# researchaccelerator-hub/distributed-crawler

Hardware: NVIDIA H100
Metric: messages/sec parsed+link-extracted+JSONL (higher is better)
Workload: dtype u8

## Files before the change

distributed_crawler_b200/csrc/kernels.cuh:

```cuda
#pragma once
#include "scalars.cuh"
#include "tg_walk.cuh"
#include "tg_lane.cuh"
#include "yt_walk.cuh"
#include "gm_walk.cuh"
#include "yt_lane.cuh"

namespace tgi {

constexpr int WARPS_PER_CTA = 8;
constexpr int CTA_THREADS = WARPS_PER_CTA * 32;
#ifndef LB_PARSE
#define LB_PARSE 6
#endif
#ifndef LB_SIZE
#define LB_SIZE 6
#endif
#ifndef LB_ESC
#define LB_ESC 6
#endif
#ifndef LB_MAPS
#define LB_MAPS 6
#endif
#ifndef LB_YT
// ... 79 lines not shown
  TgRecView v;
  const tgi_tg_rec* rec = &b.recs[r];
  v.rec = rec;
  v.text = b.strs + rec->str_off;
  v.text_len = rec->text_len;
  v.alt = v.text + v.text_len;
  v.alt_len = rec->alt_len;
  v.media = v.alt + v.alt_len;
  v.media_len = rec->media_len;
  v.handle = v.media + v.media_len;
  v.handle_len = rec->handle_len;
  v.ct = rec->content_type;
  v.flags = rec->flags;
  v.e0 = b.ent_off[r];
  v.e1 = b.ent_off[r + 1];
  return v;
}

template <bool ENTITIES>
DEVI void parse_one_record(const TgBatchDev& b, const CfgDev& cfg, const ParseOut& o, uint64_t r, TgRecView v) {
  const int l = lane_id();
  uint32_t status = TGI_ST_EMITTED, nlinks = 0, lstart = 0;
  if ((cfg.flags & TGI_CFG_HAS_MIN_POST_DATE) && (int64_t)v.rec->date < cfg.min_post_date) {
    status = TGI_ST_SKIPPED;
  } else if (v.flags & TGI_RF_PANIC) {
    status = TGI_ST_FAILED;
  } else {
    if (!ENTITIES) v.e1 = v.e0;
    uint32_t ub = warp_link_upper_bound(v, b.ents);
    if (ub >= (1u << 20)) {
      if (l == 0) atomicOr(o.err, ERR_TOO_MANY_LINKS);
      ub = 0;
    }
    if (ub) {
      if (l == 0) lstart = atomicAdd(o.cursor, ub);
      lstart = __shfl_sync(FULL, lstart, 0);
      if (lstart + ub > o.arena_cap || lstart + ub < lstart) {
        if (l == 0) atomicOr(o.err, ERR_ARENA_OVERFLOW);
      } else {
        const tgi_tg_chan* ch = &b.chans[v.rec->chan_idx];
        LinkSink ls;
        ls.out = o.arena + lstart;
        ls.cap = ub;
        ls.count = 0;
        ls.name_bytes = 0;
        ls.self = b.chan_strs + ch->str_off + ch->title_len;
        ls.self_len = ch->name_len;
        bool ok = warp_extract_links(v, b.ents, b.aux, o.ent_range, ls);
        nlinks = ls.count;
        if (!ok) {
          status = TGI_ST_FAILED;
          nlinks = 0;
        }
      }
    }
  }
  if (l == 0) {
    o.status[r] = (uint8_t)status;
    o.linelen[r] = 0;
    o.link_start[r] = lstart;
    o.link_count[r] = nlinks;
  }
}

DEVI void tg_parse_body(const TgBatchDev& b, const CfgDev& cfg, uint32_t run_flags, const ParseOut& o) {
  int wid = threadIdx.x >> 5;
  uint64_t nwarps = (uint64_t)gridDim.x * WARPS_PER_CTA;
  for (uint64_t r = (uint64_t)blockIdx.x * WARPS_PER_CTA + wid; r < b.n; r += nwarps) {
    const uint64_t rn = r + nwarps;
    unsigned long long nx_off = 0;
    uint32_t nx_len = 0;
    if (rn < b.n) {
      asm volatile("ld.global.nc.u64 %0, [%1];" : "=l"(nx_off) : "l"(&b.recs[rn].str_off));
      asm volatile("ld.global.nc.u32 %0, [%1];" : "=r"(nx_len) : "l"(&b.recs[rn].text_len));
    }
    if (b.ent_off[r + 1] == b.ent_off[r])
      parse_one_record<false>(b, cfg, o, r, load_rec_view(b, r));
    if (rn < b.n) {
      const uint32_t off = (uint32_t)lane_id() * 128u;
      if (off < nx_len + 127u && off < 2048u) asm volatile("prefetch.global.L1 [%0];" ::"l"(b.strs + nx_off + off));
    }
  }
}
__global__ void __launch_bounds__(CTA_THREADS, LB_PARSE) tg_parse_kernel(TgBatchDev b, CfgDev cfg, uint32_t run_flags, ParseOut o) { tg_parse_body(b, cfg, run_flags, o); }
DEVI void tg_ent_map_body(const TgBatchDev& b, const ParseOut& o) {
  const int wid = threadIdx.x >> 5, l = lane_id();
  const uint64_t ngroups = (b.n + 31) / 32, nwarps = (uint64_t)gridDim.x * WARPS_PER_CTA;
  for (uint64_t g = (uint64_t)blockIdx.x * WARPS_PER_CTA + wid; g < ngroups; g += nwarps) {
    const uint64_t rl = g * 32 + l;
    uint32_t todo = __ballot_sync(FULL, rl < b.n && b.ent_off[rl + 1] != b.ent_off[rl]);
    while (todo) {
      const uint64_t r = g * 32 + (uint32_t)(__ffs(todo) - 1);
      todo &= todo - 1;
      warp_map_entities(load_rec_view(b, r), b.ents, o.ent_range);
    }
  }
}
__global__ void __launch_bounds__(CTA_THREADS, LB_PARSE) tg_ent_map_kernel(TgBatchDev b, ParseOut o) { tg_ent_map_body(b, o); }
DEVI void tg_parse_ent_body(const TgBatchDev& b, const CfgDev& cfg, uint32_t run_flags, const ParseOut& o) {
  const int wid = threadIdx.x >> 5, l = lane_id();
  const uint64_t ngroups = (b.n + 31) / 32, nwarps = (uint64_t)gridDim.x * WARPS_PER_CTA;
  for (uint64_t g = (uint64_t)blockIdx.x * WARPS_PER_CTA + wid; g < ngroups; g += nwarps) {
    const uint64_t rl = g * 32 + l;
    uint32_t todo = __ballot_sync(FULL, rl < b.n && b.ent_off[rl + 1] != b.ent_off[rl]);
    while (todo) {
      const uint64_t r = g * 32 + (uint32_t)(__ffs(todo) - 1);
      todo &= todo - 1;
      parse_one_record<true>(b, cfg, o, r, load_rec_view(b, r));
    }
  }
}
__global__ void __launch_bounds__(CTA_THREADS, LB_PARSE) tg_parse_ent_kernel(TgBatchDev b, CfgDev cfg, uint32_t run_flags, ParseOut o) {
  tg_parse_ent_body(b, cfg, run_flags, o);
}

DEVI void tg_size_lane_body(const TgBatchDev& b, const CfgDev& cfg, const ParseOut& o) {
  const int wid = threadIdx.x >> 5, l = lane_id();
  const uint64_t ngroups = (b.n + 31) / 32, nwarps = (uint64_t)gridDim.x * WARPS_PER_CTA;
  uint64_t var_sum = 0;
  for (uint64_t g = (uint64_t)blockIdx.x * WARPS_PER_CTA + wid; g < ngroups; g += nwarps) {
    uint64_t r = g * 32 + l;
    bool active = r < b.n;
    if (!active) r = b.n - 1;
    active = active && o.status[r] == TGI_ST_EMITTED;
    if (!__any_sync(FULL, active)) continue;
    TgWalkArgs a;
    a.b = &b;
    a.cfg = &cfg;
    a.r = r;
    a.v = load_rec_view(b, r);
    a.links = o.arena + o.link_start[r];
    a.n_links = active ? o.link_count[r] : 0u;
    const tgi_tg_rec* rec = a.v.rec;
    const ChanDerived cd = b.chan_derived[rec->chan_idx];
    const TgDerived d = tg_derive(a, cd);
    uint32_t xl[8] = {0, 0, 0, 0, 0, 0, 0, 0};
    uint32_t tot = 0;
    bool warp_comments = false, warp_map = false;
    const uint32_t r0 = b.react_off[r], nr = b.react_off[r + 1] - r0;
    if (active && !(cfg.flags & CFGDEV_CLOCK_INVALID)) {
      uint32_t L[8] = {ndigits_i64(rec->id / 1048576), ndigits_i64(rec->chat_id), ndigits_i64(rec->view_count),
                       ndigits_i64(rec->share_count), ndigits_i64(d.ncomments), cfg.tz == 0 ? 22u : 27u, 0, 0};
      uint32_t chan[4] = {cd.user_len, cd.name_len, cd.title_len, cd.cdata_len};
      uint32_t cf[4] = {cfg.label_len, cfg.created_tg_len, cfg.created_yt_len, cfg.capture_len};
      tot = tg_size_fixed(L, chan, cf, d.has_user, d.album);
      tot += a.v.ct == TGI_CT_OTHER ? 0u : (uint32_t)kPostTypeLen[a.v.ct];
      if (a.v.ct == TGI_CT_OTHER) xl[XL_ALT] = thread_esc_len(a.v.alt, a.v.alt_len);
      if (d.has_media) xl[XL_MEDIA] = thread_esc_len(a.v.media, a.v.media_len);
      xl[XL_HANDLE] = thread_esc_len(a.v.handle, a.v.handle_len);
      if (d.comments_nil) xl[XL_COMMENTS] = 4;
      else if (d.c1 == d.c0) xl[XL_COMMENTS] = 2;
      else warp_comments = true;
      if (nr == 0) {
        xl[XL_REACTIONS] = 2;
        xl[XL_FLAGS] = XLF_SIMPLE_MAP;
      } else if (nr <= LANE_MAP_MAX) {
        uint32_t sz = 2u, live = 0;
        bool simple = true;
        for (uint32_t j = 0; j < nr; j++) {
          const tgi_reaction rc = b.reacts[r0 + j];
          const uint8_t* kp = b.aux + rc.emoji_off;
          const uint32_t el = thread_esc_len(kp, rc.emoji_len);
          simple = simple && el == rc.emoji_len && rc.emoji_len >= 1 && rc.emoji_len <= 8;
          bool last = true;
          for (uint32_t i = j + 1; i < nr; i++) {
            const tgi_reaction ri = b.reacts[r0 + i];
            if (key_cmp(b.aux + ri.emoji_off, ri.emoji_len, kp, rc.emoji_len) == 0) last = false;
          }
          if (last) {
            sz += 3u + el + ndigits_i64(rc.count);
            live++;
          }
        }
        if (simple) {
          xl[XL_REACTIONS] = sz + (live - 1u);
          xl[XL_FLAGS] = XLF_SIMPLE_MAP;
        } else {
          warp_map = true;
        }
      } else {
        warp_map = true;
      }
      if (a.n_links) {
        uint32_t s = a.n_links - 1u;
        for (uint32_t k = 0; k < a.n_links; k++) s += a.links[k].len + 2u;
        xl[XL_OUTLINKS] = s;
      }
    }
    const bool sized = active && !(cfg.flags & CFGDEV_CLOCK_INVALID);
    uint32_t todo = __ballot_sync(FULL, sized && d.desc_len != 0);
    while (todo) {
      const int src = __ffs(todo) - 1;
      todo &= todo - 1;
      const uint8_t* p = (const uint8_t*)__shfl_sync(FULL, (unsigned long long)(uintptr_t)d.desc, src);
      const uint32_t n = __shfl_sync(FULL, d.desc_len, src);
      bool ex = false;
      const uint32_t e = warp_esc_len(p, n, &ex);
      if (l == src) {
        xl[XL_DESC] = e;
        if (ex) xl[XL_FLAGS] |= XLF_DESC_EXACT;
      }
    }
    todo = __ballot_sync(FULL, warp_comments);
    while (todo) {
      const int src = __ffs(todo) - 1;
      todo &= todo - 1;
      const uint32_t e = size_tg_comments(b, __shfl_sync(FULL, d.c0, src), __shfl_sync(FULL, d.c1, src));
      if (l == src) xl[XL_COMMENTS] = e;
    }
    todo = __ballot_sync(FULL, warp_map);
    while (todo) {
      const int src = __ffs(todo) - 1;
      todo &= todo - 1;
      const uint32_t q0 = __shfl_sync(FULL, r0, src), qn = __shfl_sync(FULL, nr, src);
      uint32_t simple = 0;
      const uint32_t e = size_reaction_map(b.reacts, q0, q0 + qn, b.aux, &simple);
      if (l == src) {
        xl[XL_REACTIONS] = e;
        xl[XL_FLAGS] = (xl[XL_FLAGS] & ~XLF_SIMPLE_MAP) | (simple ? XLF_SIMPLE_MAP : 0u);
      }
    }
    if (active) {
      uint32_t var = 0;
#pragma unroll
      for (int j = 0; j < XL_COUNT; j++) var += xl[j];
      const uint32_t llen = sized ? tot + var : 0u;
      *(uint4*)(o.xlen + r * 8) = make_uint4(xl[0], xl[1], xl[2], xl[3]);
      *(uint4*)(o.xlen + r * 8 + 4) = make_uint4(xl[4], xl[5], xl[6], xl[7]);
      if (llen == 0) o.status[r] = TGI_ST_NOLINE;
      o.linelen[r] = llen;
      if (llen) var_sum += var;
    }
  }
  for (int dd = 16; dd; dd >>= 1) var_sum += __shfl_down_sync(FULL, var_sum, dd);
  if (l == 0 && var_sum) atomicAdd(o.var_total, (unsigned long long)var_sum);
}
__global__ void __launch_bounds__(CTA_THREADS, LB_SIZE) tg_size_lane_kernel(TgBatchDev b, CfgDev cfg, ParseOut o) { tg_size_lane_body(b, cfg, o); }

struct EmitIn {
  const uint8_t* status;
  const uint64_t* line_off;
  const uint32_t* link_start;
  const uint32_t* link_count;
  const uint32_t* xlen;
  uint32_t* xpos;
  const tgi_link* arena;
  uint8_t* out;
  int* err;
  uint32_t lane_text_max;
  unsigned long long* counters;
  uint32_t* list[3];
  uint32_t* list_count;
};
enum { WL_SPARSE = 0, WL_DENSE = 1, WL_MAPS = 2 };
DEVI void wl_append(uint32_t* list, uint32_t* count, bool need, uint32_t value) {
  const uint32_t m = __ballot_sync(FULL, need);
  if (!m) return;
  uint32_t base = 0;
  if (lane_id() == 0) base = atomicAdd(count, (uint32_t)__popc(m));
  base = __shfl_sync(FULL, base, 0);
  if (need) list[base + __popc(m & ((1u << lane_id()) - 1u))] = value;
}

DEVI void tg_emit_lane_body(const TgBatchDev& b, const CfgDev& cfg, const EmitIn& in, LaneShared& sh) {
  static_assert(LANE_WARPS == WARPS_PER_CTA, "one field row block per warp");
  lane_shared_fill(sh);
  __syncthreads();
  const int wid = threadIdx.x >> 5, l = lane_id();
  const uint64_t ngroups = (b.n + 31) / 32, nwarps = (uint64_t)gridDim.x * WARPS_PER_CTA;
  LaneStream s;
  ls_init(s, smem_addr(sh.stage[wid][l]));
  uint64_t bytes_out = 0, bytes_in = 0;
  for (uint64_t g = (uint64_t)blockIdx.x * WARPS_PER_CTA + wid; g < ngroups; g += nwarps) {
    uint64_t r = g * 32 + l;
    bool active = r < b.n;
    if (!active) r = b.n - 1;
    active = active && in.status[r] == TGI_ST_EMITTED;
    if (!__any_sync(FULL, active)) continue;
    uint32_t left = 0;
    emit_tg_lane(sh, sh.rows[wid][l], s, b, cfg, r, active, in.out, in.line_off, in.xlen + r * 8, in.xpos + r * 8,
                 in.arena + in.link_start[r], active ? in.link_count[r] : 0u, in.err, bytes_out, bytes_in, left);
    bool sparse = false;
    if (active && (left & 1u)) {
      const tgi_tg_rec* rec = &b.recs[r];
      const uint32_t ct = rec->content_type;
      const bool text_desc = ct == TGI_CT_TEXT || ct == TGI_CT_VIDEO || ct == TGI_CT_PHOTO || ct == TGI_CT_ANIMATION;
      const uint32_t dlen = text_desc ? ((rec->flags & TGI_RF_HAS_TEXT) ? rec->text_len : 0u) : rec->alt_len;
      sparse = esc_desc_is_sparse(in.xlen[r * 8 + XL_DESC], dlen, in.xlen[r * 8 + XL_FLAGS]);
    }
    wl_append(in.list[WL_SPARSE], in.list_count + WL_SPARSE, active && sparse, (uint32_t)r);
    wl_append(in.list[WL_DENSE], in.list_count + WL_DENSE, active && (((left & 1u) && !sparse) || (left & 0xEu)), (uint32_t)r);
    wl_append(in.list[WL_MAPS], in.list_count + WL_MAPS, active && (left & 16u), (uint32_t)r);
  }
  for (int dd = 16; dd; dd >>= 1) {
    bytes_out += __shfl_down_sync(FULL, bytes_out, dd);
    bytes_in += __shfl_down_sync(FULL, bytes_in, dd);
  }
  if (l == 0) {
    atomicAdd(in.counters, (unsigned long long)bytes_out);
    atomicAdd(in.counters + 1, (unsigned long long)bytes_in);
  }
}
#ifndef LB_LANE
#define LB_LANE 3
#endif
__global__ void __launch_bounds__(CTA_THREADS, LB_LANE) tg_emit_lane_kernel(TgBatchDev b, CfgDev cfg, EmitIn in) {
  extern __shared__ __align__(128) uint8_t lane_smem[];
  tg_emit_lane_body(b, cfg, in, *(LaneShared*)lane_smem);
}

template <int MODE>
DEVI void tg_emit_esc_body(const TgBatchDev& b, const EmitIn& in) {
  const int wid = threadIdx.x >> 5;
  const uint32_t* list = in.list[MODE == ESC_SPARSE ? WL_SPARSE : WL_DENSE];
  const uint32_t cnt = in.list_count[MODE == ESC_SPARSE ? WL_SPARSE : WL_DENSE];
  const uint32_t nwarps = gridDim.x * WARPS_PER_CTA;
  for (uint32_t i = blockIdx.x * WARPS_PER_CTA + wid; i < cnt; i += nwarps) {
    const uint64_t rr = list[i];
    TgWalkArgs a;
    a.b = &b;
    a.cfg = nullptr;
    a.r = rr;
    a.v = load_rec_view(b, rr);
    emit_tg_escapes<MODE>(in.out + in.line_off[rr], a, in.xlen + rr * 8, in.xpos + rr * 8, in.lane_text_max);
  }
}
template <int MODE>
__global__ void __launch_bounds__(CTA_THREADS, LB_ESC) tg_emit_esc_kernel(TgBatchDev b, EmitIn in) { tg_emit_esc_body<MODE>(b, in); }

DEVI void tg_emit_maps_body(const TgBatchDev& b, const EmitIn& in) {
  __shared__ MapScratch mss[WARPS_PER_CTA];
  const int wid = threadIdx.x >> 5;
  const uint32_t cnt = in.list_count[WL_MAPS], nwarps = gridDim.x * WARPS_PER_CTA;
  for (uint32_t i = blockIdx.x * WARPS_PER_CTA + wid; i < cnt; i += nwarps) {
    const uint64_t r = in.list[WL_MAPS][i];
    uint8_t* line = in.out + in.line_off[r];
    const uint32_t* xp = in.xpos + r * 8;
    const bool comments_nil = (b.recs[r].flags & TGI_RF_COMMENTS_NIL) != 0;
    const uint32_t c0 = b.comment_off[r], c1 = b.comment_off[r + 1];
    if (!comments_nil && c1 != c0) emit_tg_comments(line + xp[XL_COMMENTS], &mss[wid], b, c0, c1);
    const uint32_t r0 = b.react_off[r], r1 = b.react_off[r + 1];
    if (r1 != r0 && !(in.xlen[r * 8 + XL_FLAGS] & XLF_SIMPLE_MAP)) emit_reaction_map(line + xp[XL_REACTIONS], &mss[wid], b.reacts, r0, r1, b.aux);
    const uint32_t nl = in.link_count[r];
    if (nl > LANE_LINKS_MAX) emit_tg_outlinks(line + xp[XL_OUTLINKS], in.arena + in.link_start[r], nl);
    __syncwarp();
  }
}
__global__ void __launch_bounds__(CTA_THREADS, LB_MAPS) tg_emit_maps_kernel(TgBatchDev b, EmitIn in) { tg_emit_maps_body(b, in); }

struct YtOut {
  uint8_t* status;
  uint32_t* linelen;
  uint32_t* url_start;
  uint32_t* url_count;
  YtUrl* urls;
  uint32_t urls_cap;
  uint32_t* url_cursor;
  uint32_t* esc_len;
  uint32_t* link_start;
  uint32_t* link_count;
  tgi_link* arena;
  uint32_t arena_cap;
  uint32_t* cursor;
  int* err;
};

DEVI void yt_parse_body(const YtBatchDev& b, const CfgDev& cfg, uint32_t run_flags, const YtOut& o) {
  int wid = threadIdx.x >> 5, l = lane_id();
  uint64_t nwarps = (uint64_t)gridDim.x * WARPS_PER_CTA;
  for (uint64_t r = (uint64_t)blockIdx.x * WARPS_PER_CTA + wid; r < b.n; r += nwarps) {
    const tgi_yt_rec v = b.recs[r];
    const uint8_t* desc = b.strs + v.str_off + v.id_len + v.title_len;
    uint32_t us = 0, uc = 0, ls = 0, lc = 0;
    uint32_t ub = yt_count_http(desc, v.desc_len);
    if (ub) {
      if (l == 0) us = atomicAdd(o.url_cursor, ub);
      us = __shfl_sync(FULL, us, 0);
      if (us + ub > o.urls_cap || us + ub < us) {
        if (l == 0) atomicOr(o.err, ERR_ARENA_OVERFLOW);
      } else {
        uc = yt_extract_urls(desc, v.desc_len, o.urls + us, ub);
      }
    }
    if (run_flags & (TGI_RUN_LINKS | TGI_RUN_FRONTIER)) {
      uint32_t lb = yt_count_ytcom(desc, v.desc_len);
      if (lb >= (1u << 20)) {
        if (l == 0) atomicOr(o.err, ERR_TOO_MANY_LINKS);
        lb = 0;
      }
      if (lb) {
        if (l == 0) ls = atomicAdd(o.cursor, lb);
        ls = __shfl_sync(FULL, ls, 0);
        if (ls + lb > o.arena_cap || ls + lb < ls) {
          if (l == 0) atomicOr(o.err, ERR_ARENA_OVERFLOW);
        } else {
          lc = yt_channel_ids(desc, v.desc_len, o.arena + ls, lb);
        }
      }
    }
    if (l == 0) {
      uint8_t tmp[40];
      bool ok = !(cfg.flags & CFGDEV_CLOCK_INVALID) && cfg.created_yt_len != 0 &&
                render_time(tmp, v.published_sec, v.published_nsec, 0) != 0;
      if (ok) {
        const tgi_yt_chan& ch = b.chans[v.chan_idx];
        if (ch.cached) ok = render_time(tmp, ch.published_sec, ch.published_nsec, 0) != 0;
      }
      o.status[r] = ok ? TGI_ST_EMITTED : TGI_ST_NOLINE;
      o.linelen[r] = 0;
      o.url_start[r] = us;
      o.url_count[r] = uc;
      o.link_start[r] = ls;
      o.link_count[r] = lc;
    }
  }
}
__global__ void __launch_bounds__(CTA_THREADS, LB_YT) yt_parse_kernel(YtBatchDev b, CfgDev cfg, uint32_t run_flags, YtOut o) { yt_parse_body(b, cfg, run_flags, o); }

DEVI void yt_size_record(const YtBatchDev& b, const CfgDev& cfg, const YtOut& o, uint64_t r, YtScratch* sc) {
  const int l = lane_id();
  {
    YtArgs a;
    a.b = &b;
    a.cfg = &cfg;
    a.r = r;
    a.urls = o.urls + o.url_start[r];
    a.n_urls = o.url_count[r];
    YtSizer z;
    z.sc = sc;
    {
      const tgi_yt_rec* rec = &b.recs[r];
      const uint8_t* title = b.strs + rec->str_off + rec->id_len;
      z.el[1] = warp_esc_len(title, rec->title_len);
      z.el[0] = warp_esc_len(title + rec->title_len, rec->desc_len);
    }
    bool ok = walk_yt_record(z, a);
    if (l == 0) {
      o.esc_len[3 * r] = z.el[0];
      o.esc_len[3 * r + 1] = z.el[1];
      o.esc_len[3 * r + 2] = z.dirty ? 0u : 1u;
      o.linelen[r] = ok ? (uint32_t)z.total : 0u;
      if (!ok) o.status[r] = TGI_ST_NOLINE;
    }
  }
}
__global__ void __launch_bounds__(CTA_THREADS, LB_YT) yt_size_kernel(YtBatchDev b, CfgDev cfg, YtOut o) {
  __shared__ YtScratch scs[WARPS_PER_CTA];
  int wid = threadIdx.x >> 5;
  uint64_t nwarps = (uint64_t)gridDim.x * WARPS_PER_CTA;
  for (uint64_t r = (uint64_t)blockIdx.x * WARPS_PER_CTA + wid; r < b.n; r += nwarps) {
    if (o.status[r] != TGI_ST_EMITTED) continue;
    yt_size_record(b, cfg, o, r, &scs[wid]);
  }
}

__global__ void __launch_bounds__(CTA_THREADS, LB_YT) yt_size_lane_kernel(YtBatchDev b, CfgDev cfg, YtOut o) {
  const int wid = threadIdx.x >> 5, l = lane_id();
  const uint64_t ngroups = (b.n + 31) / 32, nwarps = (uint64_t)gridDim.x * WARPS_PER_CTA;
  for (uint64_t g = (uint64_t)blockIdx.x * WARPS_PER_CTA + wid; g < ngroups; g += nwarps) {
    uint64_t r = g * 32 + l;
    bool active = r < b.n;
    if (!active) r = b.n - 1;
    active = active && o.status[r] == TGI_ST_EMITTED;
    const tgi_yt_rec* rec = &b.recs[r];
    const uint8_t* title = b.strs + rec->str_off + rec->id_len;
    const uint32_t tn = rec->title_len, dn = rec->desc_len;
    uint32_t el0 = 0, el1 = 0;
    bool exact = false;
    uint32_t todo = __ballot_sync(FULL, active);
    while (todo) {
      const int src = __ffs(todo) - 1;
      todo &= todo - 1;
      const uint8_t* t = (const uint8_t*)__shfl_sync(FULL, (unsigned long long)(uintptr_t)title, src);
      const uint32_t a = __shfl_sync(FULL, tn, src), d = __shfl_sync(FULL, dn, src);
      bool x1 = false, x0 = false;
      const uint32_t e1 = warp_esc_len(t, a, &x1), e0 = warp_esc_len(t + a, d, &x0);
      if (l == src) {
        el0 = e0;
        el1 = e1;
        exact = x0 || x1;
      }
    }
    if (!active) continue;
    YtArgs a;
    a.b = &b;
    a.cfg = &cfg;
    a.r = r;
    a.urls = o.urls + o.url_start[r];
    a.n_urls = o.url_count[r];
    YtLaneSizer z;
    z.el[0] = el0;
    z.el[1] = el1;
    const bool ok = walk_yt_record(z, a);
    o.esc_len[3 * r] = el0;
    o.esc_len[3 * r + 1] = el1;
    o.esc_len[3 * r + 2] = !z.dirty ? 1u : (!z.small_dirty && !exact) ? 2u : 0u;
    o.linelen[r] = ok ? (uint32_t)z.total : 0u;
    if (!ok) o.status[r] = TGI_ST_NOLINE;
  }
}

DEVI void yt_emit_record(const YtBatchDev& b, const CfgDev& cfg, const YtOut& o, const uint64_t* line_off, uint8_t* out, int* err,
                         uint64_t r, YtScratch* sc) {
  YtArgs a;
  a.b = &b;
  a.cfg = &cfg;
  a.r = r;
  a.urls = o.urls + o.url_start[r];
  a.n_urls = o.url_count[r];
  YtWriter w;
  w.sc = sc;
  w.el[0] = o.esc_len[3 * r];
  w.el[1] = o.esc_len[3 * r + 1];
  w.p = out + line_off[r];
  walk_yt_record(w, a);
  if (lane_id() == 0 && (uint64_t)(w.p - out) != line_off[r + 1]) atomicOr(err, ERR_LINE_MISMATCH);
  __syncwarp();
}
__global__ void __launch_bounds__(CTA_THREADS, LB_YT) yt_emit_kernel(YtBatchDev b, CfgDev cfg, YtOut o, const uint64_t* line_off, uint8_t* out, int* err,
                                                                 int lane_mode) {
  __shared__ YtScratch scs[WARPS_PER_CTA];
  int wid = threadIdx.x >> 5, l = lane_id();
  const uint64_t ngroups = (b.n + 31) / 32, nwarps = (uint64_t)gridDim.x * WARPS_PER_CTA;
  for (uint64_t g = (uint64_t)blockIdx.x * WARPS_PER_CTA + wid; g < ngroups; g += nwarps) {
    const uint64_t rl = g * 32 + l;
    uint32_t todo = __ballot_sync(FULL, rl < b.n && o.status[rl] == TGI_ST_EMITTED && !(lane_mode && o.esc_len[3 * rl + 2]));
    while (todo) {
      const uint64_t r = g * 32 + (uint32_t)(__ffs(todo) - 1);
      todo &= todo - 1;
      yt_emit_record(b, cfg, o, line_off, out, err, r, &scs[wid]);
    }
  }
}

__global__ void __launch_bounds__(CTA_THREADS, LB_YT) yt_emit_lane_kernel(YtBatchDev b, CfgDev cfg, YtOut o, const uint64_t* line_off, uint8_t* out, int* err) {
  const int wid = threadIdx.x >> 5, l = lane_id();
  const uint64_t ngroups = (b.n + 31) / 32, nwarps = (uint64_t)gridDim.x * WARPS_PER_CTA;
  for (uint64_t g = (uint64_t)blockIdx.x * WARPS_PER_CTA + wid; g < ngroups; g += nwarps) {
    const uint64_t r = g * 32 + l;
    const bool active = r < b.n && o.status[r] == TGI_ST_EMITTED && o.esc_len[3 * r + 2];
    YtLaneWriter w;
    if (active) {
      w.el[0] = o.esc_len[3 * r];
      w.el[1] = o.esc_len[3 * r + 1];
      YtArgs a;
      a.b = &b;
      a.cfg = &cfg;
      a.r = r;
      a.urls = o.urls + o.url_start[r];
      a.n_urls = o.url_count[r];
      w.begin((uint64_t)(uintptr_t)out + line_off[r]);
      walk_yt_record(w, a);
      w.end();
      if (w.s.pos != (uint64_t)(uintptr_t)out + line_off[r + 1]) atomicOr(err, ERR_LINE_MISMATCH);
    }
    __syncwarp();
    w.flush_pending(active);
  }
}

DEVI uint64_t join_hash(long long chat, long long msg) {
  uint64_t x = (uint64_t)chat * 0x9E3779B97F4A7C15ull ^ (uint64_t)msg;
  x ^= x >> 30; x *= 0xBF58476D1CE4E5B9ull;
  x ^= x >> 27; x *= 0x94D049BB133111EBull;
  return x ^ (x >> 31);
}
__global__ void join_build_kernel(const longlong2* a, uint64_t na, uint32_t* table, uint64_t mask) {
  const uint64_t i = (uint64_t)blockIdx.x * blockDim.x + threadIdx.x;
  if (i >= na) return;
  const longlong2 k = a[i];
  for (uint64_t s = join_hash(k.x, k.y) & mask;; s = (s + 1) & mask) {
    uint32_t cur = atomicCAS(&table[s], 0u, (uint32_t)i + 1u);
    if (cur == 0) return;
    const longlong2 o = a[cur - 1];
    if (o.x == k.x && o.y == k.y) {
      atomicMin(&table[s], (uint32_t)i + 1u);
      return;
    }
  }
}
__global__ void join_probe_kernel(const longlong2* a, const uint32_t* table, uint64_t mask, const longlong2* b, uint64_t nb, long long* out) {
  const uint64_t i = (uint64_t)blockIdx.x * blockDim.x + threadIdx.x;
  if (i >= nb) return;
  const longlong2 k = b[i];
  long long res = -1;
  for (uint64_t s = join_hash(k.x, k.y) & mask;; s = (s + 1) & mask) {
    const uint32_t cur = table[s];
    if (cur == 0) break;
    const longlong2 o = a[cur - 1];
    if (o.x == k.x && o.y == k.y) {
      res = (long long)cur - 1;
      break;
    }
  }
  out[i] = res;
}

__global__ void __launch_bounds__(CTA_THREADS, 4) gm_size_kernel(GmBatchDev b, CfgDev cfg, uint8_t* status, uint32_t* linelen) {
  __shared__ YtScratch scs[WARPS_PER_CTA];
  int wid = threadIdx.x >> 5, l = lane_id();
  uint64_t nwarps = (uint64_t)gridDim.x * WARPS_PER_CTA;
  for (uint64_t r = (uint64_t)blockIdx.x * WARPS_PER_CTA + wid; r < b.n; r += nwarps) {
    YtSizer z;
    z.sc = &scs[wid];
    bool ok = walk_gm_record(z, b, cfg, r);
    if (l == 0) {
      status[r] = ok ? TGI_ST_EMITTED : TGI_ST_NOLINE;
// ... 486 lines not shown
```

distributed_crawler_b200/csrc/tg_lane.cuh:

```cuda
#pragma once
#include "tg_walk.cuh"

namespace tgi {

#ifndef LANE_STAGE
#define LANE_STAGE 256
#endif
constexpr uint32_t LANE_STAGE_BYTES = LANE_STAGE;
constexpr uint32_t LANE_STAGE_ROW = LANE_STAGE_BYTES + 16;

struct LaneStream {
  uint64_t pos;
  uint32_t c0, c1, c2, c3;
  uint32_t head;
  uint64_t seg;
  uint32_t row_s;
  uint32_t fill;
};

DEVI void ls_stage(LaneStream& s, uint64_t blk) {
  if (s.fill == 0) s.seg = blk;
  asm volatile("st.shared.v4.u32 [%0], {%1,%2,%3,%4};" ::"r"(s.row_s + s.fill), "r"(s.c0), "r"(s.c1), "r"(s.c2), "r"(s.c3) : "memory");
  s.fill += 16;
}

DEVI void ls_drain_warp(LaneStream& s) {
  if (!__any_sync(FULL, s.fill != 0)) return;
  __syncwarp();
  constexpr int LPR = LANE_STAGE_BYTES / 16, RPP = 32 / LPR;
  const int l = lane_id(), sub = l / LPR, t16 = (l % LPR) * 16;
  const uint32_t warp_rows = s.row_s - (uint32_t)l * LANE_STAGE_ROW;
#pragma unroll 2
  for (int j = 0; j < 32; j += RPP) {
    const int rj = j + sub;
    const uint32_t f = __shfl_sync(FULL, s.fill, rj);
    const uint64_t sg = __shfl_sync(FULL, s.seg, rj);
    if ((uint32_t)t16 < f) {
      uint4 w;
      asm volatile("ld.shared.v4.u32 {%0,%1,%2,%3}, [%4];" : "=r"(w.x), "=r"(w.y), "=r"(w.z), "=r"(w.w) : "r"(warp_rows + (uint32_t)rj * LANE_STAGE_ROW + (uint32_t)t16) : "memory");
      *(uint4*)(uintptr_t)(sg + (uint32_t)t16) = w;
    }
  }
  __syncwarp();
  s.fill = 0;
}
DEVI void ls_maybe_drain(LaneStream& s) {
  if (__any_sync(FULL, s.fill >= LANE_STAGE_BYTES)) ls_drain_warp(s);
}

__device__ __noinline__ void store_bytes(uint64_t blk, uint32_t c0, uint32_t c1, uint32_t c2, uint32_t c3, uint32_t lo,
                                         uint32_t hi) {
  const uint32_t w[4] = {c0, c1, c2, c3};
#pragma unroll
  for (uint32_t i = 0; i < 4; i++) {
    const uint32_t a = 4u * i;
    if (lo <= a && a + 4u <= hi) {
      *(uint32_t*)(uintptr_t)(blk + a) = w[i];
    } else {
#pragma unroll
      for (uint32_t k = 0; k < 4; k++)
        if (lo <= a + k && a + k < hi) *(uint8_t*)(uintptr_t)(blk + a + k) = (uint8_t)(w[i] >> (8u * k));
    }
  }
}

DEVI void ls_init(LaneStream& s, uint32_t row_s) {
  s.row_s = row_s;
  s.fill = 0;
  s.seg = 0;
}
DEVI void ls_begin(LaneStream& s, uint64_t addr) {
  s.pos = addr;
  s.head = (uint32_t)addr & 15u;
  s.c0 = s.c1 = s.c2 = s.c3 = 0;
}

DEVI void ls_append(LaneStream& s, uint4 w, uint32_t n) {
  const uint32_t ph = (uint32_t)s.pos & 15u, sh = (ph & 3u) * 8u;
  const uint32_t v0 = w.x << sh, v1 = __funnelshift_l(w.x, w.y, sh), v2 = __funnelshift_l(w.y, w.z, sh),
                 v3 = __funnelshift_l(w.z, w.w, sh), v4 = __funnelshift_l(w.w, 0u, sh);
  const bool b0 = (ph & 4u) != 0, b1 = (ph & 8u) != 0;
  const uint32_t z0 = b0 ? 0u : v0, z1 = b0 ? v0 : v1, z2 = b0 ? v1 : v2, z3 = b0 ? v2 : v3, z4 = b0 ? v3 : v4,
                 z5 = b0 ? v4 : 0u;
  s.c0 |= b1 ? 0u : z0;
  s.c1 |= b1 ? 0u : z1;
  s.c2 |= b1 ? z0 : z2;
  s.c3 |= b1 ? z1 : z3;
  if (ph + n >= 16u) {
    const uint64_t blk = s.pos & ~15ull;
    if (s.head == 0) {
      ls_stage(s, blk);
    } else {
      store_bytes(blk, s.c0, s.c1, s.c2, s.c3, s.head, 16u);
      s.head = 0;
    }
    s.c0 = b1 ? z2 : z4;
    s.c1 = b1 ? z3 : z5;
    s.c2 = b1 ? z4 : 0u;
    s.c3 = b1 ? z5 : 0u;
  }
  s.pos += n;
}

DEVI uint4 shr128_bytes(uint4 w, uint32_t sb) {
  const uint32_t sh = (sb & 3u) * 8u;
  const uint32_t v0 = __funnelshift_r(w.x, w.y, sh), v1 = __funnelshift_r(w.y, w.z, sh), v2 = __funnelshift_r(w.z, w.w, sh),
                 v3 = w.w >> sh;
  const bool b0 = (sb & 4u) != 0, b1 = (sb & 8u) != 0;
  const uint32_t a0 = b0 ? v1 : v0, a1 = b0 ? v2 : v1, a2 = b0 ? v3 : v2, a3 = b0 ? 0u : v3;
  return make_uint4(b1 ? a2 : a0, b1 ? a3 : a1, b1 ? 0u : a2, b1 ? 0u : a3);
}
DEVI uint4 mask128(uint4 w, uint32_t k) {
  auto m = [&](uint32_t lo) -> uint32_t {
    return k >= lo + 4u ? 0xffffffffu : (k <= lo ? 0u : (1u << ((k - lo) * 8u)) - 1u);
  };
  return make_uint4(w.x & m(0), w.y & m(4), w.z & m(8), w.w & m(12));
}

DEVI void ls_flush(LaneStream& s) {
  const uint32_t ph = (uint32_t)s.pos & 15u;
  if (ph > s.head) store_bytes(s.pos & ~15ull, s.c0, s.c1, s.c2, s.c3, s.head, ph);
  s.c0 = s.c1 = s.c2 = s.c3 = 0;
  s.head = ph;
}

DEVI void ls_skip(LaneStream& s, uint32_t g) {
  if (__any_sync(FULL, g != 0)) ls_drain_warp(s);
  if (g) {
    ls_flush(s);
    s.pos += g;
    s.head = (uint32_t)s.pos & 15u;
  }
}

constexpr int LANE_ROW_WORDS = 36;
constexpr int LANE_WARPS = 8;
constexpr uint32_t LANE_LINKS_MAX = 4;
#ifndef LANE_TEXT
#define LANE_TEXT 512
#endif
constexpr uint32_t LANE_TEXT_MAX = LANE_TEXT;
struct LaneShared {
  uint4 tmpl[kTgLaneTemplateLen / 16];
  uint4 ptype[TGI_CT__COUNT * 2];
  uint32_t pieces[64];
  uint32_t rows[LANE_WARPS][32][LANE_ROW_WORDS];
  uint4 stage[LANE_WARPS][32][LANE_STAGE_ROW / 16];
};

DEVI void lane_shared_fill(LaneShared& sh) {
  for (int i = threadIdx.x; i < kTgLaneTemplateLen / 16; i += blockDim.x) sh.tmpl[i] = ((const uint4*)kTgLaneTemplate)[i];
  for (int i = threadIdx.x; i < kTgLaneNPieces; i += blockDim.x) sh.pieces[i] = kTgLanePieces[i];
  uint32_t* pt = (uint32_t*)sh.ptype;
  for (int i = threadIdx.x; i < TGI_CT__COUNT * 8; i += blockDim.x) {
    const int ct = i >> 3, w = i & 7;
    pt[i] = w < 7 ? ((const uint32_t*)kPostType[ct])[w] : 0u;
  }
}

DEVI void emit_tg_lane(LaneShared& sh, uint32_t* row, LaneStream& s, const TgBatchDev& b, const CfgDev& cfg, uint64_t r, bool active,
                       uint8_t* out, const uint64_t* line_off, const uint32_t* xlen_g, uint32_t* xpos_g, const tgi_link* links,
                       uint32_t nl, int* err, uint64_t& bytes_out, uint64_t& bytes_in, uint32_t& left) {
  uint32_t gaps = 0, copied = 0;
  left = 0;
  TgWalkArgs a;
  a.b = &b;
  a.cfg = &cfg;
  a.r = r;
  a.links = nullptr;
  a.n_links = 0;
  {
    const tgi_tg_rec* rec = &b.recs[r];
    a.v.rec = rec;
    a.v.text = b.strs + rec->str_off;
    a.v.text_len = rec->text_len;
    a.v.alt = a.v.text + a.v.text_len;
    a.v.alt_len = rec->alt_len;
    a.v.media = a.v.alt + a.v.alt_len;
    a.v.media_len = rec->media_len;
    a.v.handle = a.v.media + a.v.media_len;
    a.v.handle_len = rec->handle_len;
    a.v.ct = rec->content_type;
    a.v.flags = rec->flags;
    a.v.e0 = a.v.e1 = 0;
  }
  const tgi_tg_rec* rec = a.v.rec;
  const ChanDerived cd = b.chan_derived[rec->chan_idx];
  const TgDerived d = tg_derive(a, cd);
  const uint32_t condmask = active ? tg_condmask(a, d) : 0u;
  const uint32_t ct = a.v.ct;

  uint8_t* rb = (uint8_t*)row;
#pragma unroll
  for (int k = 0; k < 8; k++) ((uint4*)row)[k] = make_uint4(0, 0, 0, 0);
#pragma unroll 1
  for (int f = 0; f < 5; f++) {
    const int64_t v = f == 0 ? rec->id / 1048576
                             : f == 1 ? rec->chat_id
                                      : f == 2 ? (int64_t)rec->view_count : f == 3 ? (int64_t)rec->share_count : d.ncomments;
    const uint32_t fo = f ? 16u + (f >= 2 ? 16u * f : 0u) : 0u;
    rb[128 + f] = (uint8_t)render_i64(rb + fo, v);
  }
  rb[128 + F_TIME] = (uint8_t)render_time(rb + 96, rec->date, 0, cfg.tz);

  const uint64_t line_start = (uint64_t)(uintptr_t)out + line_off[r];
  const uint32_t total = (uint32_t)(line_off[r + 1] - line_off[r]);
  ls_begin(s, active ? line_start : 0ull);

  uint32_t p = 0, t = 0;
  uint32_t multi_n = 0, multi_max = 0;
  uint32_t map_nr = 0;
  uint64_t prev = 0;
  while (p < (uint32_t)kTgLaneNPieces) {
    const uint32_t en = sh.pieces[p];
    const uint32_t kind = en & 15u, arg = (en >> 4) & 15u;
    const bool on = ((condmask >> ((en >> 8) & 15u)) & 1u) != 0;
    const uint8_t* src = nullptr;
    uint32_t n = 0, g = 0;
    bool more = false, padded = true;
    if (kind == K_LIT) {
      src = (const uint8_t*)(sh.tmpl + ((en >> 12) & 0x7FFu));
      n = on ? en >> 23 : 0u;
    } else if (kind == K_FIELD) {
      src = rb + (arg ? 16u + (arg >= 2 ? 16u * arg : 0u) : 0u);
      n = on ? rb[128 + arg] : 0u;
    } else if (kind == K_POSTTYPE) {
      src = (const uint8_t*)(sh.ptype + 2u * ct);
      n = on ? kPostTypeLen[ct] : 0u;
    } else if (kind == K_CHAN) {
      const uint32_t o = arg == 0 ? 0u : arg == 1 ? pad16(cd.user_len) : arg == 2 ? pad16(cd.user_len) + pad16(cd.name_len)
                                                             : pad16(cd.user_len) + pad16(cd.name_len) + pad16(cd.title_len);
      src = b.chan_blob + cd.off + o;
      n = !on ? 0u : arg == 0 ? cd.user_len : arg == 1 ? cd.name_len : arg == 2 ? cd.title_len : cd.cdata_len;
      copied += n;
    } else if (kind == K_CFG) {
      src = cfg.blob + (arg == 0 ? cfg.off[0] : arg == 1 ? cfg.off[1] : arg == 2 ? cfg.off[2] : cfg.off[3]);
      n = !on ? 0u : arg == 0 ? cfg.label_len : arg == 1 ? cfg.created_tg_len : arg == 2 ? cfg.created_yt_len : cfg.capture_len;
      copied += n;
    } else if (kind == K_ESC) {
      const uint8_t* sp = arg == XL_DESC ? d.desc : arg == XL_MEDIA ? a.v.media : arg == XL_HANDLE ? a.v.handle : a.v.alt;
      const uint32_t sn = arg == XL_DESC ? d.desc_len : arg == XL_MEDIA ? a.v.media_len : arg == XL_HANDLE ? a.v.handle_len : a.v.alt_len;
      uint32_t xl = 0;
      if (active) {
        xpos_g[arg] = (uint32_t)(s.pos - line_start);
        if (on) xl = xlen_g[arg];
      }
      const bool mine = on && xl == sn && sn <= LANE_TEXT_MAX;
      g = mine ? 0u : xl;
      if (g) left |= 1u << arg;
      if (mine) {
        src = sp;
        n = sn;
        copied += sn;
      }
      padded = false;
    } else if (kind == K_COMMENTS) {
      const bool mine = on && (d.comments_nil || d.c1 == d.c0);
      if (active) {
        xpos_g[XL_COMMENTS] = (uint32_t)(s.pos - line_start);
        if (on && !mine) g = xlen_g[XL_COMMENTS];
      }
      if (mine) {
        *(uint4*)(rb + 96) = make_uint4(d.comments_nil ? 0x6c6c756eu : 0x5d5bu, 0, 0, 0);
        src = rb + 96;
        n = d.comments_nil ? 4u : 2u;
      }
    } else if (kind == K_REACTIONS) {
      uint4* ent = (uint4*)row;
      uint8_t* sc = rb + 96;
      if (t == 0) {
        const uint32_t r0 = b.react_off[r], nr = b.react_off[r + 1] - r0;
        bool mine = false;
        if (active) {
          xpos_g[XL_REACTIONS] = (uint32_t)(s.pos - line_start);
          mine = on && (nr == 0 || (xlen_g[XL_FLAGS] & XLF_SIMPLE_MAP));
          if (on && !mine) g = xlen_g[XL_REACTIONS];
        }
        const uint32_t nn = mine ? nr : 0u;
        map_nr = nn;
        const uint32_t nmax = __reduce_max_sync(FULL, nn);
        for (uint32_t j = 0; j < nmax; j++) {
          if (j < nn) {
            const tgi_reaction rc = b.reacts[r0 + j];
            const uint8_t* kp = b.aux + rc.emoji_off;
            const uint32_t kl = rc.emoji_len;
            uint32_t k0 = ld_u32_unaligned(kp), k1 = kl > 4 ? ld_u32_unaligned(kp + 4) : 0u;
            if (kl < 4) k0 &= (1u << (8u * kl)) - 1u;
            if (kl > 4 && kl < 8) k1 &= (1u << (8u * (kl - 4u))) - 1u;
            ent[j] = make_uint4(k0, k1, (uint32_t)rc.count, kl);
          }
        }
        uint32_t live = 0;
        for (uint32_t j = 0; j < nmax; j++) {
          if (j < nn) {
            const uint4 e = ent[j];
            bool last = true;
            for (uint32_t i = j + 1; i < nn; i++) {
              const uint4 f = ent[i];
              if (f.x == e.x && f.y == e.y && f.w == e.w) last = false;
            }
            live += last ? 1u : 0u;
          }
        }
        multi_n = live;
        multi_max = __reduce_max_sync(FULL, multi_n);
        if (mine) {
          *(uint4*)sc = make_uint4(multi_n ? 0x7bu : 0x7d7bu, 0, 0, 0);
          src = sc;
          n = multi_n ? 1u : 2u;
        }
        prev = 0;
      } else if (t <= multi_n) {
        uint4 be = make_uint4(0, 0, 0, 0);
        uint64_t best = ~0ull;
        for (uint32_t j = 0; j < LANE_MAP_MAX; j++) {
          if (j < map_nr) {
            const uint4 e = ent[j];
            const uint64_t ck = ((uint64_t)__byte_perm(e.x, 0, 0x0123) << 32) | __byte_perm(e.y, 0, 0x0123);
            if (ck > prev && ck <= best) {
              best = ck;
              be = e;
            }
          }
        }
        prev = best;
        const uint32_t kl = be.w;
        *(uint4*)sc = make_uint4(0x22u | (be.x << 8), (be.x >> 24) | (be.y << 8), be.y >> 24, 0);
        *(uint4*)(sc + 16) = make_uint4(0, 0, 0, 0);
        sc[1 + kl] = '"';
        sc[2 + kl] = ':';
        const uint32_t dl = (uint32_t)render_i64(sc + 3 + kl, (int64_t)(int32_t)be.z);
        sc[3 + kl + dl] = t == multi_n ? '}' : ',';
        src = sc;
        n = 4u + kl + dl;
      }
      more = t < multi_max;
      padded = false;
    } else {
      if (t == 0) {
        const bool mine = on && nl <= LANE_LINKS_MAX;
        if (active) {
          xpos_g[XL_OUTLINKS] = (uint32_t)(s.pos - line_start);
          if (on && !mine) g = xlen_g[XL_OUTLINKS];
        }
        multi_n = mine ? nl : 0u;
        multi_max = __reduce_max_sync(FULL, multi_n);
      }
      if (t < multi_n) {
        const uint32_t* lw = (const uint32_t*)(links + t);
        const uint32_t len = links[t].len, lead = t ? 2u : 1u;
        uint8_t* sc = rb;
        sc[0] = t ? ',' : '"';
        sc[1] = '"';
#pragma unroll 1
        for (uint32_t k = 0; k < len; k += 4) {
          const uint32_t w = __ldg(lw + (k >> 2));
          sc[lead + k] = (uint8_t)w;
          sc[lead + k + 1] = (uint8_t)(w >> 8);
          sc[lead + k + 2] = (uint8_t)(w >> 16);
          sc[lead + k + 3] = (uint8_t)(w >> 24);
        }
        sc[lead + len] = '"';
        src = sc;
        n = lead + len + 1u;
      }
      more = t + 1 < multi_max;
      padded = false;
    }
    if (g && kind != K_ESC) left |= 16u;
    ls_skip(s, g);
    gaps += g;
    {
      const uint32_t s0 = (uint32_t)(uintptr_t)src & 15u;
      const uint4* A = (const uint4*)(src - s0);
      const uint32_t steps = __reduce_max_sync(FULL, n ? (s0 + n + 15u) >> 4 : 0u);
      uint32_t rem = n, first = s0;
      for (uint32_t i = 0; i < steps; i++, A++) {
        if (rem) {
          uint4 w = *A;
          if (first) w = shr128_bytes(w, first);
          const uint32_t k = min(rem, 16u - first);
          if (k < 16u && !padded) w = mask128(w, k);
          ls_append(s, w, k);
          rem -= k;
          first = 0;
        }
        ls_maybe_drain(s);
      }
    }
    if (more) {
      t++;
    } else {
      p++;
      t = 0;
    }
  }
  ls_flush(s);
  ls_drain_warp(s);
  if (active) {
    if ((uint32_t)(s.pos - line_start) != total) atomicOr(err, ERR_LINE_MISMATCH);
    bytes_out += total - gaps;
    bytes_in += copied;
  }
}

}
```

Measured before the change: 184.2 million.

## Restructure lane stream drain and source copy paths with shared-row metadata

Drain now stores each row's segment address and fill level in shared memory and reads them back, instead of two warp shuffles per row. The number of drain iterations is sized to the largest fill rather than a fixed count. Piece copies are split into a shared-memory path (aligned, no shift or mask) and a global path using __ldg, with phase bits computed once per piece instead of on every append. The partial-block store helper is inlined, link scratch is zero-padded so masking can be dropped, and the lane kernel's launch bound drops from 3 to 2 blocks per SM. This trades occupancy for more registers and less per-step overhead.

```diff
diff --git a/distributed_crawler_b200/csrc/kernels.cuh b/distributed_crawler_b200/csrc/kernels.cuh
--- a/distributed_crawler_b200/csrc/kernels.cuh
+++ b/distributed_crawler_b200/csrc/kernels.cuh
@@ -405,7 +405,7 @@
   }
 }
 #ifndef LB_LANE
-#define LB_LANE 3
+#define LB_LANE 2
 #endif
 __global__ void __launch_bounds__(CTA_THREADS, LB_LANE) tg_emit_lane_kernel(TgBatchDev b, CfgDev cfg, EmitIn in) {
   extern __shared__ __align__(128) uint8_t lane_smem[];
diff --git a/distributed_crawler_b200/csrc/tg_lane.cuh b/distributed_crawler_b200/csrc/tg_lane.cuh
--- a/distributed_crawler_b200/csrc/tg_lane.cuh
+++ b/distributed_crawler_b200/csrc/tg_lane.cuh
@@ -24,32 +24,36 @@
   s.fill += 16;
 }
 
-DEVI void ls_drain_warp(LaneStream& s) {
-  if (!__any_sync(FULL, s.fill != 0)) return;
+DEVI void ls_drain_rows(LaneStream& s, uint32_t lg) {
+  asm volatile("st.shared.v4.u32 [%0], {%1,%2,%3,%4};" ::"r"(s.row_s + LANE_STAGE_BYTES), "r"((uint32_t)s.seg),
+               "r"((uint32_t)(s.seg >> 32)), "r"(s.fill), "r"(0u) : "memory");
   __syncwarp();
-  constexpr int LPR = LANE_STAGE_BYTES / 16, RPP = 32 / LPR;
-  const int l = lane_id(), sub = l / LPR, t16 = (l % LPR) * 16;
-  const uint32_t warp_rows = s.row_s - (uint32_t)l * LANE_STAGE_ROW;
+  const uint32_t l = (uint32_t)lane_id(), sub = l >> lg, t16 = (l & ((1u << lg) - 1u)) * 16u, rpp = 32u >> lg;
+  const uint32_t rows = s.row_s - l * LANE_STAGE_ROW;
 #pragma unroll 2
-  for (int j = 0; j < 32; j += RPP) {
-    const int rj = j + sub;
-    const uint32_t f = __shfl_sync(FULL, s.fill, rj);
-    const uint64_t sg = __shfl_sync(FULL, s.seg, rj);
-    if ((uint32_t)t16 < f) {
-      uint4 w;
-      asm volatile("ld.shared.v4.u32 {%0,%1,%2,%3}, [%4];" : "=r"(w.x), "=r"(w.y), "=r"(w.z), "=r"(w.w) : "r"(warp_rows + (uint32_t)rj * LANE_STAGE_ROW + (uint32_t)t16) : "memory");
-      *(uint4*)(uintptr_t)(sg + (uint32_t)t16) = w;
+  for (uint32_t j = 0; j < (1u << lg); j++) {
+    const uint32_t row = rows + (j * rpp + sub) * LANE_STAGE_ROW;
+    uint32_t sl, sh, f, z;
+    asm volatile("ld.shared.v4.u32 {%0,%1,%2,%3}, [%4];" : "=r"(sl), "=r"(sh), "=r"(f), "=r"(z) : "r"(row + LANE_STAGE_BYTES) : "memory");
+    if (t16 < f) {
+      uint32_t x, y, w;
+      asm volatile("ld.shared.v4.u32 {%0,%1,%2,%3}, [%4];" : "=r"(x), "=r"(y), "=r"(z), "=r"(w) : "r"(row + t16) : "memory");
+      asm volatile("st.global.v4.u32 [%0], {%1,%2,%3,%4};" ::"l"((((uint64_t)sh << 32) | sl) + t16), "r"(x), "r"(y), "r"(z), "r"(w)
+                   : "memory");
     }
   }
   __syncwarp();
   s.fill = 0;
 }
+DEVI void ls_drain_warp(LaneStream& s) {
+  const uint32_t fmax = __reduce_max_sync(FULL, s.fill);
+  if (fmax) ls_drain_rows(s, 32u - __clz((fmax >> 4) - 1u));
+}
 DEVI void ls_maybe_drain(LaneStream& s) {
-  if (__any_sync(FULL, s.fill >= LANE_STAGE_BYTES)) ls_drain_warp(s);
-}
-
-__device__ __noinline__ void store_bytes(uint64_t blk, uint32_t c0, uint32_t c1, uint32_t c2, uint32_t c3, uint32_t lo,
-                                         uint32_t hi) {
+  if (__any_sync(FULL, s.fill >= LANE_STAGE_BYTES)) ls_drain_rows(s, 31u - __clz(LANE_STAGE_BYTES >> 4));
+}
+
+DEVI void store_block_bytes(uint64_t blk, uint32_t c0, uint32_t c1, uint32_t c2, uint32_t c3, uint32_t lo, uint32_t hi) {
   const uint32_t w[4] = {c0, c1, c2, c3};
 #pragma unroll
   for (uint32_t i = 0; i < 4; i++) {
@@ -63,9 +67,13 @@
     }
   }
 }
+__device__ __noinline__ void store_bytes(uint64_t blk, uint32_t c0, uint32_t c1, uint32_t c2, uint32_t c3, uint32_t lo,
+                                         uint32_t hi) {
+  store_block_bytes(blk, c0, c1, c2, c3, lo, hi);
+}
 
 DEVI void ls_init(LaneStream& s, uint32_t row_s) {
-  s.row_s = row_s;
+  asm volatile("mov.b32 %0, %1;" : "=r"(s.row_s) : "r"(row_s));
   s.fill = 0;
   s.seg = 0;
 }
@@ -75,11 +83,20 @@
   s.c0 = s.c1 = s.c2 = s.c3 = 0;
 }
 
-DEVI void ls_append(LaneStream& s, uint4 w, uint32_t n) {
-  const uint32_t ph = (uint32_t)s.pos & 15u, sh = (ph & 3u) * 8u;
+struct LanePhase {
+  uint32_t ph, sh;
+  bool b0, b1;
+};
+DEVI LanePhase ls_phase(const LaneStream& s) {
+  const uint32_t ph = (uint32_t)s.pos & 15u;
+  return {ph, (ph & 3u) * 8u, (ph & 4u) != 0, (ph & 8u) != 0};
+}
+
+DEVI void ls_append(LaneStream& s, const LanePhase& q, uint4 w, uint32_t n) {
+  const uint32_t ph = q.ph, sh = q.sh;
   const uint32_t v0 = w.x << sh, v1 = __funnelshift_l(w.x, w.y, sh), v2 = __funnelshift_l(w.y, w.z, sh),
                  v3 = __funnelshift_l(w.z, w.w, sh), v4 = __funnelshift_l(w.w, 0u, sh);
-  const bool b0 = (ph & 4u) != 0, b1 = (ph & 8u) != 0;
+  const bool b0 = q.b0, b1 = q.b1;
   const uint32_t z0 = b0 ? 0u : v0, z1 = b0 ? v0 : v1, z2 = b0 ? v1 : v2, z3 = b0 ? v2 : v3, z4 = b0 ? v3 : v4,
                  z5 = b0 ? v4 : 0u;
   s.c0 |= b1 ? 0u : z0;
@@ -91,7 +108,7 @@
     if (s.head == 0) {
       ls_stage(s, blk);
     } else {
-      store_bytes(blk, s.c0, s.c1, s.c2, s.c3, s.head, 16u);
+      store_block_bytes(blk, s.c0, s.c1, s.c2, s.c3, s.head, 16u);
       s.head = 0;
     }
     s.c0 = b1 ? z2 : z4;
@@ -119,7 +136,7 @@
 
 DEVI void ls_flush(LaneStream& s) {
   const uint32_t ph = (uint32_t)s.pos & 15u;
-  if (ph > s.head) store_bytes(s.pos & ~15ull, s.c0, s.c1, s.c2, s.c3, s.head, ph);
+  if (ph > s.head) store_block_bytes(s.pos & ~15ull, s.c0, s.c1, s.c2, s.c3, s.head, ph);
   s.c0 = s.c1 = s.c2 = s.c3 = 0;
   s.head = ph;
 }
@@ -215,26 +232,27 @@
     const uint32_t en = sh.pieces[p];
     const uint32_t kind = en & 15u, arg = (en >> 4) & 15u;
     const bool on = ((condmask >> ((en >> 8) & 15u)) & 1u) != 0;
-    const uint8_t* src = nullptr;
+    const uint4* ssrc = (const uint4*)rb;
+    const uint8_t* gsrc = nullptr;
     uint32_t n = 0, g = 0;
-    bool more = false, padded = true;
+    bool more = false;
     if (kind == K_LIT) {
-      src = (const uint8_t*)(sh.tmpl + ((en >> 12) & 0x7FFu));
+      ssrc = sh.tmpl + ((en >> 12) & 0x7FFu);
       n = on ? en >> 23 : 0u;
     } else if (kind == K_FIELD) {
-      src = rb + (arg ? 16u + (arg >= 2 ? 16u * arg : 0u) : 0u);
+      ssrc = (const uint4*)rb + (arg ? 1u + (arg >= 2 ? arg : 0u) : 0u);
       n = on ? rb[128 + arg] : 0u;
     } else if (kind == K_POSTTYPE) {
-      src = (const uint8_t*)(sh.ptype + 2u * ct);
+      ssrc = sh.ptype + 2u * ct;
       n = on ? kPostTypeLen[ct] : 0u;
     } else if (kind == K_CHAN) {
       const uint32_t o = arg == 0 ? 0u : arg == 1 ? pad16(cd.user_len) : arg == 2 ? pad16(cd.user_len) + pad16(cd.name_len)
                                                              : pad16(cd.user_len) + pad16(cd.name_len) + pad16(cd.title_len);
-      src = b.chan_blob + cd.off + o;
+      gsrc = b.chan_blob + cd.off + o;
       n = !on ? 0u : arg == 0 ? cd.user_len : arg == 1 ? cd.name_len : arg == 2 ? cd.title_len : cd.cdata_len;
       copied += n;
     } else if (kind == K_CFG) {
-      src = cfg.blob + (arg == 0 ? cfg.off[0] : arg == 1 ? cfg.off[1] : arg == 2 ? cfg.off[2] : cfg.off[3]);
+      gsrc = cfg.blob + (arg == 0 ? cfg.off[0] : arg == 1 ? cfg.off[1] : arg == 2 ? cfg.off[2] : cfg.off[3]);
       n = !on ? 0u : arg == 0 ? cfg.label_len : arg == 1 ? cfg.created_tg_len : arg == 2 ? cfg.created_yt_len : cfg.capture_len;
       copied += n;
     } else if (kind == K_ESC) {
@@ -248,12 +266,11 @@
       const bool mine = on && xl == sn && sn <= LANE_TEXT_MAX;
       g = mine ? 0u : xl;
       if (g) left |= 1u << arg;
+      gsrc = sp;
       if (mine) {
-        src = sp;
         n = sn;
         copied += sn;
       }
-      padded = false;
     } else if (kind == K_COMMENTS) {
       const bool mine = on && (d.comments_nil || d.c1 == d.c0);
       if (active) {
@@ -262,7 +279,7 @@
       }
       if (mine) {
         *(uint4*)(rb + 96) = make_uint4(d.comments_nil ? 0x6c6c756eu : 0x5d5bu, 0, 0, 0);
-        src = rb + 96;
+        ssrc = (const uint4*)(rb + 96);
         n = d.comments_nil ? 4u : 2u;
       }
     } else if (kind == K_REACTIONS) {
@@ -306,7 +323,7 @@
         multi_max = __reduce_max_sync(FULL, multi_n);
         if (mine) {
           *(uint4*)sc = make_uint4(multi_n ? 0x7bu : 0x7d7bu, 0, 0, 0);
-          src = sc;
+          ssrc = (const uint4*)sc;
           n = multi_n ? 1u : 2u;
         }
         prev = 0;
@@ -331,11 +348,10 @@
         sc[2 + kl] = ':';
         const uint32_t dl = (uint32_t)render_i64(sc + 3 + kl, (int64_t)(int32_t)be.z);
         sc[3 + kl + dl] = t == multi_n ? '}' : ',';
-        src = sc;
+        ssrc = (const uint4*)sc;
         n = 4u + kl + dl;
       }
       more = t < multi_max;
-      padded = false;
     } else {
       if (t == 0) {
         const bool mine = on && nl <= LANE_LINKS_MAX;
@@ -350,6 +366,8 @@
         const uint32_t* lw = (const uint32_t*)(links + t);
         const uint32_t len = links[t].len, lead = t ? 2u : 1u;
         uint8_t* sc = rb;
+#pragma unroll
+        for (int k = 0; k < 3; k++) ((uint4*)sc)[k] = make_uint4(0, 0, 0, 0);
         sc[0] = t ? ',' : '"';
         sc[1] = '"';
 #pragma unroll 1
@@ -361,29 +379,37 @@
           sc[lead + k + 3] = (uint8_t)(w >> 24);
         }
         sc[lead + len] = '"';
-        src = sc;
         n = lead + len + 1u;
       }
       more = t + 1 < multi_max;
-      padded = false;
     }
     if (g && kind != K_ESC) left |= 16u;
     ls_skip(s, g);
     gaps += g;
     {
-      const uint32_t s0 = (uint32_t)(uintptr_t)src & 15u;
-      const uint4* A = (const uint4*)(src - s0);
+      const bool global = kind == K_CHAN || kind == K_CFG || kind == K_ESC;
+      const uint32_t s0 = global ? (uint32_t)(uintptr_t)gsrc & 15u : 0u;
+      const uint4* A = global ? (const uint4*)(gsrc - s0) : nullptr;
       const uint32_t steps = __reduce_max_sync(FULL, n ? (s0 + n + 15u) >> 4 : 0u);
       uint32_t rem = n, first = s0;
-      for (uint32_t i = 0; i < steps; i++, A++) {
+      LanePhase q = ls_phase(s);
+      for (uint32_t i = 0; i < steps; i++) {
+        if (global && i == 1) q = ls_phase(s);
         if (rem) {
-          uint4 w = *A;
-          if (first) w = shr128_bytes(w, first);
-          const uint32_t k = min(rem, 16u - first);
-          if (k < 16u && !padded) w = mask128(w, k);
-          ls_append(s, w, k);
+          uint4 w;
+          uint32_t k;
+          if (global) {
+            w = __ldg(A + i);
+            if (first) w = shr128_bytes(w, first);
+            k = min(rem, 16u - first);
+            if (k < 16u && kind == K_ESC) w = mask128(w, k);
+            first = 0;
+          } else {
+            w = ssrc[i];
+            k = min(rem, 16u);
+          }
+          ls_append(s, q, w, k);
           rem -= k;
-          first = 0;
         }
         ls_maybe_drain(s);
       }
```

Result: faster. 189.3 million, median of 6 (+2.8%).
